# ToniChopp/ECAMP

Hardware: AMD Instinct MI355X
Metric: pretrain image-report pairs/sec (ViT-B/16, 224^2, seq=128) (higher is better)
Workload: dtype bf16

## Files before the change

### ecamp_amd/csrc/gemm.hip

```cpp
#include "common.h"
#include <stdlib.h>
#include <string.h>
#include <stdint.h>
#include <map>
#include <string>
#include <vector>

#include "gemm_args.h"
#include "gemm_q8.h"
#include "gemm_q16.h"

#define BM 128
#define BN 128
#define BK 64

__device__ __forceinline__ int swz(int row) { return (row >> 1) & 7; }

__device__ __forceinline__ void g2r_kc(const bf16_t* P, long ld, int row0, int nrows, int k0, int kend, int tid,
                                       uint4 (&r)[4]) {
#pragma unroll
    for (int i = 0; i < 4; ++i) {
        int c = tid + 256 * i;
        int row = c >> 3, kc = c & 7;
        int gr = row0 + row, gk = k0 + kc * 8;
// ... 856 lines not shown
    if (prof) ecamp_prof_end(stream);
    if (q8_out && !q8) {
        const long n4 = M * N / 4;
        int nb = (int)((n4 + 255) / 256);
        if (nb > 4096) nb = 4096;
        hipLaunchKernelGGL(quant_fp8_delayed_kernel<bf16_t>, dim3(nb), dim3(256), 0, stream, (const bf16_t*)C, q8_scale, (unsigned int*)q8_out, q8_amax_slots, n4);
    }
    ECAMP_LAUNCH_CHECK();
    return 0;
}

struct WgTile { int prob, m0, n0, first, count; };
struct WgRedProb { float* C; long ldc; int M, N; float alpha; int accumulate; const float* alpha_dev; };
struct WgRedArgs { const WgTile* tiles; const float* slabs; int ntiles, pad; WgRedProb p[4]; };
__global__ __launch_bounds__(256) void wgrad_group_reduce_kernel(WgRedArgs a) {
    const int t = blockIdx.x >> 4, chunk = blockIdx.x & 15;
    const WgTile T = a.tiles[t];
    const WgRedProb P = T.prob == 0 ? a.p[0] : T.prob == 1 ? a.p[1] : T.prob == 2 ? a.p[2] : a.p[3];
    const float al = P.alpha_dev ? P.alpha * P.alpha_dev[0] : P.alpha;
#pragma unroll
    for (int j = 0; j < 4; ++j) {
        const int idx = chunk * 1024 + j * 256 + threadIdx.x;
        const int r = idx >> 6, c = (idx & 63) * 4;
        const int gm = T.m0 + r, gn = T.n0 + c;
        if (gm >= P.M || gn >= P.N) continue;
        const float4* src = reinterpret_cast<const float4*>(a.slabs + (long)T.first * 65536) + idx;
        float4 acc = src[0];
        for (int z = 1; z < T.count; ++z) {
            const float4 p = src[(long)z * 16384];
            acc.x += p.x; acc.y += p.y; acc.z += p.z; acc.w += p.w;
        }
        float* c_ = P.C + (long)gm * P.ldc + gn;
        float4 o = P.accumulate ? *reinterpret_cast<float4*>(c_) : make_float4(0.f, 0.f, 0.f, 0.f);
        o.x += al * acc.x; o.y += al * acc.y; o.z += al * acc.z; o.w += al * acc.w;
        *reinterpret_cast<float4*>(c_) = o;
    }
}

struct WgPlan {
    std::vector<Q8ItemRec> items;
    std::vector<int> first;
    std::vector<WgTile> tiles;
    int nitems = 0, nwg = 0, ntiles = 0;
    size_t off_first = 0, off_tiles = 0, bytes = 0;
};
static std::map<std::string, WgPlan> g_wg_plans;

static long wg_tiles(int n, const int64_t* n_out, const int64_t* k_in) {
    long tiles = 0;
    for (int p = 0; p < n; ++p) tiles += (long)ceil_div(n_out[p], 256) * ceil_div(k_in[p], 256);
    return tiles;
}

static const WgPlan* wg_plan(int n, const int64_t* n_out, const int64_t* k_in, const unsigned* has_bias, int64_t rows, int ncu) {
    const int reserve = ecamp_opt(OPT_P8_WGRAD_RESERVE);
    std::string key((const char*)n_out, n * sizeof(int64_t));
    key.append((const char*)k_in, n * sizeof(int64_t)).append((const char*)has_bias, n * sizeof(unsigned)).append((const char*)&rows, 8).append((const char*)&ncu, 4);
    key.append((const char*)&reserve, sizeof(int));
    auto it = g_wg_plans.find(key);
    if (it != g_wg_plans.end()) return &it->second;
    const long KT = (rows + 63) / 64;
    WgPlan pl;
    std::vector<WgTile>& tiles = pl.tiles;
    for (int p = 0; p < n; ++p)
        for (int mb = 0; mb < ceil_div(n_out[p], 256); ++mb)
            for (int nb = 0; nb < ceil_div(k_in[p], 256); ++nb) tiles.push_back({p, mb * 256, nb * 256, 0, 0});
    std::vector<Q8ItemRec>& items = pl.items;
    std::vector<int>& first = pl.first;
    const int plan_mode = ecamp_opt(OPT_WGRAD_PLAN);
    const long T = (long)tiles.size();
    const int cap = p8_bwd_cus();
    long S = (ncu + T / 2) / T;
    while (S > 1 && (T * S > cap || KT / S < 4)) --S;
    if (plan_mode == 1 && S >= 1 && T * S >= ncu / 2 && T * S <= cap) {
        const long P = T * S;
        for (long t = 0; t < T; ++t) { tiles[t].first = (int)(t * S); tiles[t].count = (int)S; }
        std::vector<long> order(P);
        for (long j = 0; j < P; ++j) order[j] = j;
        const long q8 = P / 8, r8 = P % 8;
        for (long w = 0; w < P; ++w) {
            const long xcd = w % 8, slot = w / 8;
            const long j = (xcd < r8 ? xcd * (q8 + 1) : r8 * (q8 + 1) + (xcd - r8) * q8) + slot;
            const long seg = order[j] / T, t = order[j] % T;
            const long k0 = KT * seg / S, k1 = KT * (seg + 1) / S;
            const long kend = k1 * 64 < rows ? k1 * 64 : rows;
            WgTile& Tt = tiles[t];
            first.push_back((int)items.size());
            items.push_back({Tt.prob, Tt.m0, Tt.n0, (int)(k0 * 64), (int)kend, (int)(t * S + seg), (Tt.n0 == 0 && has_bias[Tt.prob]) ? 1 : 0, 0});
        }
    } else {
    const long U = KT / 2;
    const long units = (long)tiles.size() * U;
    long q = (units + ncu - 1) / ncu;
    if (q < 1) q = 1;
    long u = 0;
    while (u < units) {
        first.push_back((int)items.size());
        long take = q < units - u ? q : units - u;
        while (take > 0) {
            const long t = u / U, j0 = u % U, len = take < U - j0 ? take : U - j0;
            WgTile& T = tiles[t];
            if (T.count == 0) T.first = (int)items.size();
            ++T.count;
            const long k0 = 2 * j0, k1 = j0 + len == U ? KT : 2 * (j0 + len);
            const long kend = k1 * 64 < rows ? k1 * 64 : rows;
            items.push_back({T.prob, T.m0, T.n0, (int)(k0 * 64), (int)kend, (int)items.size(), (T.n0 == 0 && has_bias[T.prob]) ? 1 : 0, 0});
            u += len; take -= len;
        }
    }
    }
    first.push_back((int)items.size());
    pl.nitems = (int)items.size(); pl.nwg = (int)first.size() - 1; pl.ntiles = (int)tiles.size();
    pl.off_first = items.size() * sizeof(Q8ItemRec);
    pl.off_tiles = pl.off_first + (first.size() * sizeof(int) + 31) / 32 * 32;
    pl.bytes = pl.off_tiles + tiles.size() * sizeof(WgTile);
    return &(g_wg_plans[key] = std::move(pl));
}
static int wg_ncu() {
    const int env = ecamp_opt(OPT_WGRAD_GROUP_CUS), ncu = p8_num_cu();
    if (env > 0) return env < ncu ? env : ncu;
    const int bwd = p8_bwd_cus(), q = ncu * 3 / 4;
    return bwd < q ? bwd : q;
}
extern "C" int ecamp_wgrad_group_supported(int32_t n, const int64_t* n_out, const int64_t* k_in, int64_t rows) {
    if (n < 1 || n > 4 || !n_out || !k_in || rows < 256) return 0;
    for (int p = 0; p < n; ++p) {
        if (n_out[p] % 8 || k_in[p] % 8 || n_out[p] <= 0 || k_in[p] <= 0) return 0;
        if (rows * n_out[p] * 2 > LIM_2GB || rows * k_in[p] * 2 > LIM_2GB) return 0;
    }
    return wg_tiles(n, n_out, k_in) >= 16 ? 1 : 0;
}
extern "C" int64_t ecamp_wgrad_group_workspace_bytes(int32_t n, const int64_t* n_out, const int64_t* k_in, int64_t rows) {
    if (!ecamp_wgrad_group_supported(n, n_out, k_in, rows)) return 0;
    return (wg_tiles(n, n_out, k_in) + p8_num_cu() + 1) * 262144;
}
extern "C" int ecamp_wgrad_group_workgroups(int32_t workgroups) {
    if (workgroups > 0) return workgroups < p8_num_cu() ? workgroups : p8_num_cu();
    return wg_ncu();
}
extern "C" int64_t ecamp_wgrad_group_table_bytes(int32_t n, const int64_t* n_out, const int64_t* k_in, int64_t rows) {
    if (!ecamp_wgrad_group_supported(n, n_out, k_in, rows)) return 0;
    const long tiles = wg_tiles(n, n_out, k_in), ncu = p8_num_cu();
    return (tiles + ncu + 1) * (long)sizeof(Q8ItemRec) + ((ncu + 2) * 4 + 31) / 32 * 32 + tiles * (long)sizeof(WgTile) + 64;
}
extern "C" int64_t ecamp_wgrad_group_table(int32_t n, const int64_t* n_out, const int64_t* k_in, const int32_t* has_bias, int64_t rows,
                                           int32_t workgroups, void* host_table) {
    if (!n_out || !k_in || !has_bias || !host_table || !ecamp_wgrad_group_supported(n, n_out, k_in, rows))
        return ecamp_set_error(-1, "wgrad_group_table: unsupported group or null pointer");
    unsigned hb[4] = {0, 0, 0, 0};
    for (int p = 0; p < n; ++p) hb[p] = has_bias[p] ? 1u : 0u;
    const WgPlan* pl = wg_plan(n, n_out, k_in, hb, rows, ecamp_wgrad_group_workgroups(workgroups));
    char* out = (char*)host_table;
    memcpy(out, pl->items.data(), pl->items.size() * sizeof(Q8ItemRec));
    memcpy(out + pl->off_first, pl->first.data(), pl->first.size() * sizeof(int));
    memcpy(out + pl->off_tiles, pl->tiles.data(), pl->tiles.size() * sizeof(WgTile));
    return (int64_t)pl->bytes;
}
extern "C" int ecamp_wgrad_group(int32_t n, const void* const* dy, const void* const* x, float* const* gw, float* const* gb, const int64_t* n_out,
                                 const int64_t* k_in, int64_t rows, float alpha, const float* alpha_dev, const int32_t* accumulate, float* ws,
                                 const void* table, int64_t table_bytes, int32_t workgroups, hipStream_t stream) {
    ECAMP_CHECK_ARG(dy && x && gw && gb && n_out && k_in && accumulate && ws && table, "wgrad_group: null pointer");
    ECAMP_CHECK_ARG(((uintptr_t)table & 31) == 0, "wgrad_group: the item table must be 32-byte aligned");
    ECAMP_CHECK_ARG(ecamp_wgrad_group_supported(n, n_out, k_in, rows), "wgrad_group: unsupported group (1-4 layers, rows >= 256, dims %% 8 == 0, < 2 GB operands)");
    unsigned hb[4] = {0, 0, 0, 0};
    bool any_bias = false;
    for (int p = 0; p < n; ++p) {
        ECAMP_CHECK_ARG(dy[p] && x[p] && gw[p], "wgrad_group: null operand");
        ECAMP_CHECK_ARG(((uintptr_t)dy[p] & 15) == 0 && ((uintptr_t)x[p] & 15) == 0 && ((uintptr_t)gw[p] & 15) == 0, "wgrad_group: operands must be 16-byte aligned");
        hb[p] = gb[p] ? 1u : 0u;
        any_bias = any_bias || gb[p];
    }
    const int nwg = ecamp_wgrad_group_workgroups(workgroups);
    const WgPlan* pl = wg_plan(n, n_out, k_in, hb, rows, nwg);
    ECAMP_CHECK_ARG(table_bytes == (int64_t)pl->bytes, "wgrad_group: the item table (%ld bytes) was not built for the current plan (%ld bytes: CU reserve "
                    "or workgroup count changed since ecamp_wgrad_group_table) -- rebuild it", (long)table_bytes, (long)pl->bytes);
    const char* tb = (const char*)table;
    Q8Group G;
    memset(&G, 0, sizeof(G));
    G.items = (const Q8ItemRec*)tb; G.wg_first = (const int*)(tb + pl->off_first); G.slabs = ws; G.nprob = n;
    WgRedArgs R;
    memset(&R, 0, sizeof(R));
    R.tiles = (const WgTile*)(tb + pl->off_tiles); R.slabs = ws; R.ntiles = pl->ntiles;
    for (int p = 0; p < n; ++p) {
        G.p[p].A = dy[p]; G.p[p].B = x[p]; G.p[p].lda = n_out[p]; G.p[p].ldb = k_in[p]; G.p[p].M = (int)n_out[p]; G.p[p].N = (int)k_in[p];
        G.p[p].rowsum = gb[p]; G.p[p].alpha_out = alpha; G.p[p].alpha_dev_out = alpha_dev;
        R.p[p].C = gw[p]; R.p[p].ldc = k_in[p]; R.p[p].M = (int)n_out[p]; R.p[p].N = (int)k_in[p]; R.p[p].alpha = alpha; R.p[p].alpha_dev = alpha_dev;
        R.p[p].accumulate = accumulate[p];
    }
    GemmArgs g = gemm_args(dy[0], x[0], ws, n_out[0], k_in[0], rows, n_out[0], k_in[0], k_in[0]);
    g.out_f32 = 1; g.alpha_out = alpha; g.nbm = 1; g.nbn = 1; g.wide = 1; g.partial = ws;
    typedef void (*q8i_fn)(GemmArgs, Q8Group);
    const bool lean = (ecamp_opt(OPT_Q8_SCH) & 8) != 0;
    const bool four = q16_wgrad_on(Q16W_GROUPED);
    const q8i_fn fn = four ? (any_bias ? (q8i_fn)gemm_bf16_q16_wgrad_items_kernel<true> : (q8i_fn)gemm_bf16_q16_wgrad_items_kernel<false>)
                    : any_bias ? (lean ? (q8i_fn)gemm_bf16_q8_items_kernel<true, 1> : (q8i_fn)gemm_bf16_q8_items_kernel<true, 0>)
                               : (lean ? (q8i_fn)gemm_bf16_q8_items_kernel<false, 1> : (q8i_fn)gemm_bf16_q8_items_kernel<false, 0>);
    double work = 0.0;
    for (int p = 0; p < n; ++p) work += 2.0 * (double)n_out[p] * (double)k_in[p] * (double)rows;
    const bool prof = ecamp_prof_active();
    if (prof) {
        char tag[40];
        snprintf(tag, sizeof tag, "%s:w:n%d:%ld:%ld:%ld:wg%d", four ? "grp16" : "grp", n, (long)rows, (long)n_out[0], (long)k_in[0], pl->nwg);
        ecamp_prof_begin(ECAMP_PROF_GEMM_BF16, work, stream, tag);
    }
    launch_persistent(fn, (long)pl->nwg, (long)pl->nwg, four ? 256 : 512, stream, g, G);
    g_q8_launches += n;
    if (four) ++g_q16_launches;
    ++g_wg_launches;
    hipLaunchKernelGGL(wgrad_group_reduce_kernel, dim3(pl->ntiles * 16), dim3(256), 0, stream, R);
    if (prof) ecamp_prof_end(stream);
    ECAMP_LAUNCH_CHECK();
    return 0;
}
```

### ecamp_amd/functions.py

```python
import math
import os

import torch

from . import hip_ops as ops


def _none(n):
    return (None,) * n


_BLOCK = None


class _wgrad_block:

    def __init__(self, arena):
        self.arena, self.items, self.ready, self.prev = arena, [], [], None

    def __enter__(self):
        global _BLOCK
        self.prev, _BLOCK = _BLOCK, self
        self.outer_ready, self.arena.deferred = self.arena.deferred, self.ready
        return self

    def collect(self, item):
        self.items.append(item)
        if len(self.items) == 4:
            self.issue()

    def issue(self):
        _issue(self.items)
        del self.items[:]

    def __exit__(self, et, ev, tb):
        global _BLOCK
        _BLOCK, self.arena.deferred = self.prev, self.outer_ready
        if et is None:
            self.issue()
            if self.ready:
                self.arena.ready(*self.ready)
        return False


def _issue(items, workgroups=0):
    if len(items) >= 2 and ops.wgrad_group_supported(items):
        ops.wgrad_group_async(items, workgroups=workgroups)
    else:
        for dy, x, gw, gb, acc in items:
            ops.linear_wgrad_async(dy, x, gw, gb=gb, accumulate=acc)


_MLM_CHUNK_ROWS = int(os.environ.get("ECAMP_MLM_CHUNK_ROWS", "0"))


def _wgrad(A, dy, x, w, gb=None, alpha_dev=None, shape=None):
    gw, acc = A.gradw(w, shape)
    if _BLOCK is not None and _BLOCK.arena is A and alpha_dev is None:
        _BLOCK.collect((dy, x, gw, gb, acc))
        return
    ops.linear_wgrad_async(dy, x, gw, alpha_dev=alpha_dev, gb=gb, accumulate=acc)


def _f8_site(m, x, weights):
    if not (m.fp8_forward and x.dtype == torch.bfloat16):
        return None
    _, sc, am, cal = m.arena.f8_site(weights)
    return (sc, am) if cal else None


def _dense(m, x, weights, bias, shape=None, x8=None, next_w=None, **kw):
    A = m.arena
    plist = list(weights) if isinstance(weights, (list, tuple)) else [weights]
    if m.fp8_forward and x.dtype == torch.bfloat16:
        i, sc, am, cal = A.f8_site(plist)
        if x8 is None:
            x8 = ops.quantize_fp8_site(x, sc, am, cal)
            A.f8_cal.add(i)
        w8, ws = A.w8(plist, shape)
        if next_w is not None:
            _, nsc, nam, ncal = A.f8_site(next_w)
            if ncal:
                return ops.gemm_fp8(x8, sc, w8, ws, bias, q8_site=(nsc, nam), **kw)
            return ops.gemm_fp8(x8, sc, w8, ws, bias, **kw) + (None,)
        return ops.gemm_fp8(x8, sc, w8, ws, bias, **kw)
    w = A.fused_w(plist, shape) if len(plist) > 1 else A.w(plist[0])
    r = ops.linear_fwd(x, w, bias, **kw)
    return r + (None,) if next_w is not None else r


def _vit_linear(m, x, lin, x8=None, next_w=None, residual=None, **kw):
    if residual is not None and residual.dtype != x.dtype:
        return ops.linear_fwd_res32(x, m.arena.w(lin.weight), lin.bias.data, residual)
    return _dense(m, x, lin.weight, lin.bias.data, x8=x8, next_w=next_w, residual=residual, **kw)


def f32_carrier(x32, dtype):
    assert x32.dim() == 2 and x32.dtype == torch.float32 and x32.is_contiguous()
    return x32.view(dtype)[:, 0::2]


def f32_stream(x):
    if x.dtype == torch.float32:
        return x
    M, D = x.shape
    assert x.stride() == (2 * D, 2) and x.storage_offset() % 2 == 0, "not an f32 residual-stream carrier"
    return x.new_empty(0, dtype=torch.float32).set_(x.untyped_storage(), x.storage_offset() // 2, (M, D), (D, 1))


def _ln_bwd(dy, z, mean, rstd, gamma, ggamma, gbeta, dres=None):
    if z.dtype != dy.dtype:
# ... 410 lines not shown
    A.ready(ln.weight, ln.bias, out.dense.weight, out.dense.bias, inter.dense.weight, inter.dense.bias)
    return dx


class BertLayerFn(torch.autograd.Function):
    @staticmethod
    def forward(ctx, h, layer, m, B, S, key_mask, pa, ph):
        tape = []
        a, a8 = _self_attn_fwd(m, layer.attention.self, layer.attention.output, h, B, S, key_mask, pa, ph, tape, next_w=layer.intermediate.dense.weight)
        o = _ffn_fwd(m, layer.intermediate, layer.output, a, ph, tape, x8=a8)
        ctx.s = (tape, m, B, S, key_mask, pa, ph)
        return o

    @staticmethod
    def backward(ctx, do):
        tape, m, B, S, key_mask, pa, ph = ctx.s
        with _wgrad_block(m.arena):
            da = _ffn_bwd(m, tape[1], do.contiguous(), ph)
            dh = _self_attn_bwd(m, tape[0], da, B, S, key_mask, pa, ph)
        ctx.s = None
        return (dh,) + _none(7)


class FusionFn(torch.autograd.Function):

    @staticmethod
    def forward(ctx, e, lat, gap, fl, m, B, S, T, key_mask, pa, ph):
        A = m.arena
        H = e.shape[1]
        heads = m.bert_config.num_attention_heads
        hd = H // heads
        tape = []
        a1 = _self_attn_fwd(m, fl.attention.self, fl.attention.output, e, B, S, key_mask, pa, ph, tape)
        ca = fl.cross_self_attention
        q = _dense(m, a1, ca.query.weight, ca.query.bias.data)
        bkv = A.fused_f32([ca.key.bias, ca.value.bias], (2 * H,))
        kv = _dense(m, lat, [ca.key.weight, ca.value.weight], bkv, shape=(2 * H, H))
        f = kv.view(-1)
        qs, ks = (S * H, H, hd), (T * 2 * H, 2 * H, hd)
        s1, o1 = m.next_rng()
        c, lse, cbits = ops.attn_fwd(q, f[2 * H:], f[3 * H:], B, heads, S, T - 1, hd, qs, ks, ks, 1.0 / math.sqrt(hd), None, pa, s1, o1, want_mask=True)
        gp = ops.linear_fwd(gap, A.w(fl.gap_mlp.weight), fl.gap_mlp.bias.data)
        c2 = ops.bcast_add(c, gp).view(B * S, H)
        ol = fl.out_layer
        y = _dense(m, c2, ol.dense.weight, ol.dense.bias.data)
        s2, o2 = m.next_rng()
        a2, z, mean, rstd, a28 = _ln_fwd(m, y, ol.LayerNorm, fl.intermediate.dense.weight, residual=a1, drop_p=ph, seed=s2, offset=o2)
        out = _ffn_fwd(m, fl.intermediate, fl.output, a2, ph, tape, x8=a28)
        ctx.s = (tape, e, lat, gap, fl, m, B, S, T, key_mask, pa, ph, a1, q, kv, c, lse, c2, z, mean, rstd, (s1, o1), (s2, o2), cbits)
        return out

    @staticmethod
    def backward(ctx, dout):
        (tape, e, lat, gap, fl, m, B, S, T, key_mask, pa, ph, a1, q, kv, c, lse, c2, z, mean, rstd, (s1, o1), (s2, o2), cbits) = ctx.s
        A = m.arena
        G = A.grad
        H = e.shape[1]
        heads = m.bert_config.num_attention_heads
        hd = H // heads
        da2 = _ffn_bwd(m, tape[1], dout.contiguous(), ph)
        ol = fl.out_layer
        ln = ol.LayerNorm
        dz, dy = _post_ln_bwd(m, da2, z, mean, rstd, ln, ph, s2, o2)
        _wgrad(A, dy, c2, ol.dense.weight, gb=G(ol.dense.bias))
        dc2 = ops.linear_dgrad(dy, A.w(ol.dense.weight))
        dgp = ops.seq_sum(dc2.view(B, S, H), 0, S, 1.0)
        gm = fl.gap_mlp
        _wgrad(A, dgp, gap, gm.weight, gb=G(gm.bias))
        dgap = ops.linear_dgrad(dgp, A.w(gm.weight))
        ca = fl.cross_self_attention
        dq = torch.empty_like(q)
        dkv = ops.zeros(kv.shape, kv.device, kv.dtype)
        f, df = kv.view(-1), dkv.view(-1)
        qs, ks = (S * H, H, hd), (T * 2 * H, 2 * H, hd)
        ops.attn_bwd(q, f[2 * H:], f[3 * H:], c, dc2.view(B, S, H), lse, dq, df[2 * H:], df[3 * H:], B, heads, S, T - 1, hd, qs, ks, ks,
                     qs, ks, ks, 1.0 / math.sqrt(hd), None, pa, s1, o1, drop_bits=cbits)
        _wgrad(A, dkv, lat, [ca.key.weight, ca.value.weight], shape=(2 * H, H), gb=A.fused_grad([ca.key.bias, ca.value.bias], (2 * H,)))
        dlat = ops.linear_dgrad(dkv, A.fused_w([ca.key.weight, ca.value.weight], (2 * H, H)))
        _wgrad(A, dq, a1, ca.query.weight, gb=G(ca.query.bias))
        da1 = ops.linear_dgrad(dq, A.w(ca.query.weight), residual=dz)
        A.ready(ln.weight, ln.bias, ol.dense.weight, ol.dense.bias, gm.weight, gm.bias, ca.query.weight, ca.query.bias,
                ca.key.weight, ca.key.bias, ca.value.weight, ca.value.bias)
        de = _self_attn_bwd(m, tape[0], da1, B, S, key_mask, pa, ph)
        ctx.s = None
        return (de, dlat, dgap) + _none(8)


def _mlm_transform(m, h, pr):
    fp8 = m.fp8_forward and m.fp8_head
    if fp8:
        t1, pre = _dense(m, h, pr.transform.dense.weight, pr.transform.dense.bias.data, act=1, save_pre=True)
    else:
        t1, pre = ops.linear_fwd(h, m.arena.w(pr.transform.dense.weight), pr.transform.dense.bias.data, act=1, save_pre=True)
    t, _, mean, rstd, t8 = _ln_fwd(m, t1, pr.transform.LayerNorm, pr.decoder.weight if fp8 else None)
    return t1, pre, mean, rstd, t, t8


def _mlm_decoder(m, t, t8, pr):
    if m.fp8_forward and m.fp8_head:
        return _dense(m, t, pr.decoder.weight, pr.bias.data, x8=t8)
    return ops.linear_fwd(t, m.arena.w(pr.decoder.weight), pr.bias.data)


def mlm_head_eval(h, labels, weights, cls, m, ids=None, rows_hint=None, compact=False):
    from .data import MASK
    pr = cls.predictions
    M = h.shape[0]
    labels, weights = labels.view(-1), weights.view(-1)
    ids = ids.view(-1) if ids is not None else None
    m._eval_found = m._aux_mlm_rows = None
    if compact:
        V = pr.decoder.weight.shape[0]
        if rows_hint is None:
            h, labels, weights, rows, found = ops.compact_rows(h, labels, weights, ids, MASK, V, cap=M)
            cap = ops.compact_cap(found.item())
            if cap <= M:
                h, labels, weights, rows = h[:cap], labels[:cap], weights[:cap], rows[:cap]
        else:
            h, labels, weights, rows, found = ops.compact_rows(h, labels, weights, ids, MASK, V, cap=ops.compact_cap(rows_hint))
        m._eval_found = found
        if m.keep_aux:
# ... 131 lines not shown
```

### ecamp_amd/hip_ops.py

```python
import ctypes
import os

import torch

from . import _lib, streams
from ._lib import BF16, F32, call

_I64x3 = ctypes.c_int64 * 3


def code(dtype):
    if dtype == torch.float32:
        return F32
    if dtype == torch.bfloat16 or dtype == torch.float16:
        want = "bf16" if dtype == torch.bfloat16 else "f16"
        if _lib.half() != want:
            raise TypeError("a %s tensor reached the %s build of libecamp_hip -- call ecamp_amd._lib.set_half(%r) first "
                            "(ECAMP(compute_dtype=...) does)" % (dtype, _lib.half(), want))
        return BF16
    raise TypeError("ecamp_amd supports float32, bfloat16 and float16 activations, got %s" % dtype)


def _chk(*ts):
    for t in ts:
# ... 91 lines not shown
        return y, pre, y8
    return (y, pre) if save_pre else y


def linear_fwd_fp8(x, w8, w_scale, bias=None, act=0, residual=None, save_pre=False):
    M, K = x.shape
    N = w8.shape[0]
    assert w8.shape[1] == K and w8.dtype == torch.uint8 and x.dtype == torch.bfloat16 and x.is_contiguous() and w8.is_contiguous()
    x8, xs = quantize_fp8(x)
    y = torch.empty((M, N), device=x.device, dtype=torch.bfloat16)
    pre = torch.empty((M, N), device=x.device, dtype=torch.bfloat16) if save_pre else None
    call("ecamp_gemm_fp8", ptr(x8), ptr(w8), ptr(y), M, N, K, K, K, N, ptr(xs), ptr(w_scale), ptr(bias), ptr(residual),
         residual.stride(0) if residual is not None else 0, ptr(pre), N, int(act), ptr(None), ptr(None), ptr(None), stream())
    return (y, pre) if save_pre else y


def linear_dgrad(dy, w, gmul=None, alpha=1.0, alpha_dev=None, residual=None, gmul_is_grad=False):
    M, N = dy.shape
    K = w.shape[1]
    dx = torch.empty((M, K), device=dy.device, dtype=dy.dtype)
    gemm(dy, w, dx, M, K, N, True, dy.stride(0), False, w.stride(0), K, gmul=gmul, ldg=gmul.stride(0) if gmul is not None else 0,
         residual=residual, ldr=residual.stride(0) if residual is not None else 0, alpha=alpha, alpha_dev=alpha_dev,
         act=2 if (gmul_is_grad and gmul is not None) else 0)
    return dx


_SPLIT_CACHE = {}
_WG_TABLES = {}


def set_option(name, value):
    call("ecamp_set_option", name.encode(), int(value))
    _SPLIT_CACHE.clear()
    _WG_TABLES.clear()


def _split_k(n_out, k_in, m, dtype=torch.bfloat16):
    key = (n_out, k_in, m, dtype)
    s = _SPLIT_CACHE.get(key)
    if s is None:
        s = _SPLIT_CACHE[key] = max(1, int(_lib.load().ecamp_gemm_suggest_split(n_out, k_in, m, 0, 0, code(dtype))))
    return s


def linear_wgrad(dy, x, gw, alpha=1.0, alpha_dev=None, gb=None, accumulate=True):
    M, N = dy.shape
    K = x.shape[1]
    assert gw.dtype == torch.float32 and gw.is_contiguous() and gw.numel() == N * K
    gemm(dy, x, gw, N, K, M, False, dy.stride(0), False, x.stride(0), K, alpha=alpha, alpha_dev=alpha_dev, out_f32=True,
         accumulate=bool(accumulate), split_k=_split_k(N, K, M, dy.dtype), rowsum=gb)


WGRAD_GROUP = os.environ.get("ECAMP_WGRAD_GROUP", "1") != "0"


def wgrad_group_supported(items):
    if not WGRAD_GROUP or not 1 <= len(items) <= 4:
        return False
    rows = items[0][0].shape[0]
    for dy, x, gw, gb, _ in items:
        if dy.dtype not in (torch.bfloat16, torch.float16) or x.dtype != dy.dtype or dy.shape[0] != rows or x.shape[0] != rows:
            return False
        if not (dy.is_contiguous() and x.is_contiguous() and gw.is_contiguous() and gw.dtype == torch.float32):
            return False
    n = len(items)
    no = (ctypes.c_int64 * n)(*[it[0].shape[1] for it in items])
    ki = (ctypes.c_int64 * n)(*[it[1].shape[1] for it in items])
    return bool(_lib.load().ecamp_wgrad_group_supported(n, ctypes.cast(no, ctypes.c_void_p), ctypes.cast(ki, ctypes.c_void_p), rows))


def _wgrad_group_table(dev, n, no, ki, hb, rows, workgroups):
    lib = _lib.load()
    nwg = int(lib.ecamp_wgrad_group_workgroups(int(workgroups)))
    key = (str(dev), tuple(no), tuple(ki), tuple(hb), int(rows), nwg)
    t = _WG_TABLES.get(key)
    if t is None:
        cv = lambda a: ctypes.cast(a, ctypes.c_void_p)
        cap = int(lib.ecamp_wgrad_group_table_bytes(n, cv(no), cv(ki), rows))
        host = torch.empty((cap,), dtype=torch.uint8)
        used = int(lib.ecamp_wgrad_group_table(n, cv(no), cv(ki), cv((ctypes.c_int32 * n)(*hb)), rows, int(workgroups), ctypes.c_void_p(host.data_ptr())))
        if used <= 0:
            raise _lib.EcampHipError("ecamp_wgrad_group_table failed: %s" % lib.ecamp_last_error().decode())
        t = _WG_TABLES[key] = host[:used].to(dev)
    return t


def wgrad_group(items, alpha=1.0, alpha_dev=None, workgroups=0):
    n = len(items)
    rows = items[0][0].shape[0]
    no = (ctypes.c_int64 * n)(*[it[0].shape[1] for it in items])
    ki = (ctypes.c_int64 * n)(*[it[1].shape[1] for it in items])
    vp = lambda ts: (ctypes.c_void_p * n)(*[t.data_ptr() if t is not None else None for t in ts])
    dyp, xp, gwp, gbp = vp([it[0] for it in items]), vp([it[1] for it in items]), vp([it[2] for it in items]), vp([it[3] for it in items])
    acc = (ctypes.c_int32 * n)(*[1 if it[4] else 0 for it in items])
    cv = lambda a: ctypes.cast(a, ctypes.c_void_p)
    dev = items[0][0].device
    table = _wgrad_group_table(dev, n, no, ki, [1 if it[3] is not None else 0 for it in items], rows, workgroups)
    nws = int(_lib.load().ecamp_wgrad_group_workspace_bytes(n, cv(no), cv(ki), rows)) // 4
    ws = torch.empty((nws,), device=dev, dtype=torch.float32)
    call("ecamp_wgrad_group", n, cv(dyp), cv(xp), cv(gwp), cv(gbp), cv(no), cv(ki), rows, float(alpha), ptr(alpha_dev), cv(acc), ptr(ws), ptr(table),
         table.numel(), int(workgroups), stream())


def colsum(x, out, alpha=1.0, period=0, lo=0, hi=0, alpha_dev=None):
    _chk(x, out)
    M, N = x.shape
    call("ecamp_colsum", ptr(x), x.stride(0), M, N, float(alpha), ptr(alpha_dev), period, lo, hi, ptr(out), code(x.dtype), stream())


def layernorm_fwd(x, gamma, beta, eps, residual=None, drop_p=0.0, seed=0, offset=0, q8_site=None):
    _chk(x, gamma, beta)
    rows, cols = x.shape
    assert x.is_contiguous()
    y = torch.empty_like(x)
    mean = torch.empty(rows, device=x.device, dtype=torch.float32)
    rstd = torch.empty(rows, device=x.device, dtype=torch.float32)
    fused = residual is not None or drop_p > 0.0
    z = torch.empty_like(x) if fused else None
    if q8_site is not None:
        y8 = torch.empty((rows, cols), device=x.device, dtype=torch.uint8)
        call("ecamp_layernorm_fwd_q8", ptr(x), ptr(residual), ptr(z), ptr(gamma), ptr(beta), ptr(y), ptr(mean), ptr(rstd), rows, cols,
             float(eps), float(drop_p), seed, offset, ptr(y8), ptr(q8_site[0]), ptr(q8_site[1]), code(x.dtype), stream())
        return y, (z if fused else x), mean, rstd, y8
    call("ecamp_layernorm_fwd", ptr(x), ptr(residual), ptr(z), ptr(gamma), ptr(beta), ptr(y), ptr(mean), ptr(rstd), rows, cols,
         float(eps), float(drop_p), seed, offset, code(x.dtype), stream())
    return y, (z if fused else x), mean, rstd


def layernorm_bwd(dy, z, mean, rstd, gamma, ggamma, gbeta, dres=None, drop_p=0.0, seed=0, offset=0, want_drop=False):
    rows, cols = dy.shape
    assert dy.is_contiguous() and z.is_contiguous()
    dz = torch.empty_like(dy)
    dxd = torch.empty_like(dy) if want_drop else None
    call("ecamp_layernorm_bwd", ptr(dy), ptr(z), ptr(mean), ptr(rstd), ptr(gamma), ptr(dres), ptr(dz), ptr(dxd), ptr(ggamma),
         ptr(gbeta), rows, cols, float(drop_p), seed, offset, code(dy.dtype), stream())
    return (dz, dxd) if want_drop else dz


def layernorm_fwd_x32(x, gamma, beta, eps, dtype):
    _chk(x, gamma, beta)
    rows, cols = x.shape
    assert x.is_contiguous() and x.dtype == torch.float32
    y = torch.empty((rows, cols), device=x.device, dtype=dtype)
    mean = torch.empty(rows, device=x.device, dtype=torch.float32)
    rstd = torch.empty(rows, device=x.device, dtype=torch.float32)
    call("ecamp_layernorm_fwd_x32", ptr(x), ptr(gamma), ptr(beta), ptr(y), ptr(mean), ptr(rstd), rows, cols, float(eps), code(dtype), stream())
    return y, x, mean, rstd


def layernorm_bwd_z32(dy, z, mean, rstd, gamma, ggamma, gbeta, dres=None):
    rows, cols = dy.shape
    assert dy.is_contiguous() and z.is_contiguous() and z.dtype == torch.float32 and (dres is None or dres.dtype == dy.dtype)
    dz = torch.empty_like(dy)
    call("ecamp_layernorm_bwd_z32", ptr(dy), ptr(z), ptr(mean), ptr(rstd), ptr(gamma), ptr(dres), ptr(dz), ptr(ggamma), ptr(gbeta), rows, cols,
# ... 544 lines not shown
```

### include/ecamp_hip.h

```cpp
#ifndef ECAMP_HIP_H
#define ECAMP_HIP_H
#include <stdint.h>
#ifdef __cplusplus
extern "C" {
#endif

typedef struct ihipStream_t* ecampStream_t;

#define ECAMP_F32 0
#define ECAMP_BF16 1

#define ECAMP_ABI_VERSION 5
int ecamp_abi_version(void);
const char* ecamp_last_error(void);
int ecamp_half_format(void);

int ecamp_gemm(const void* A, const void* B, void* C, int64_t M, int64_t N, int64_t K, int a_kc, int64_t lda, int b_kc,
               int64_t ldb, int64_t ldc, const float* bias, const void* residual, int64_t ldr, void* pre_out, int64_t ldp,
               const void* gmul, int64_t ldg, int act, float alpha, const float* alpha_dev, int dtype, int out_f32, int accumulate,
               int split_k, float* splitk_ws, float* rowsum, ecampStream_t stream);
int ecamp_gemm_res32(const void* A, const void* B, float* C, int64_t M, int64_t N, int64_t K, int64_t lda, int64_t ldb, int64_t ldc,
                     const float* bias, const float* residual, int64_t ldr, int dtype, ecampStream_t stream);
int ecamp_gemm_suggest_split(int64_t M, int64_t N, int64_t K, int a_kc, int b_kc, int dtype);
int ecamp_wgrad_group_supported(int32_t n, const int64_t* n_out, const int64_t* k_in, int64_t rows);
int64_t ecamp_wgrad_group_workspace_bytes(int32_t n, const int64_t* n_out, const int64_t* k_in, int64_t rows);
int64_t ecamp_wgrad_group_table_bytes(int32_t n, const int64_t* n_out, const int64_t* k_in, int64_t rows);
int64_t ecamp_wgrad_group_table(int32_t n, const int64_t* n_out, const int64_t* k_in, const int32_t* has_bias, int64_t rows,
                                int32_t workgroups, void* host_table);
int ecamp_wgrad_group_workgroups(int32_t workgroups);
int ecamp_wgrad_group(int32_t n, const void* const* dy, const void* const* x, float* const* gw, float* const* gb, const int64_t* n_out,
                      const int64_t* k_in, int64_t rows, float alpha, const float* alpha_dev, const int32_t* accumulate, float* ws,
                      const void* table, int64_t table_bytes, int32_t workgroups, ecampStream_t stream);
int64_t ecamp_gemm_workspace_bytes(int64_t M, int64_t N, int64_t K, int32_t split_k);
int64_t ecamp_attn_bwd_workspace_bytes(int32_t B, int32_t H, int32_t Tq);
int64_t ecamp_sr_bwd_workspace_bytes(void);
int ecamp_set_option(const char* name, int32_t value);

int ecamp_amax(const void* x, float* out, int64_t n, int32_t dtype, ecampStream_t stream);
int ecamp_quant_fp8_delayed(const void* x, const float* scale, void* q, float* amax_slots, int64_t n, int32_t dtype, ecampStream_t stream);
int ecamp_fp8_roll(float* amax_slots, float* scale, int32_t n, float* hist, int32_t hist_len, int32_t hist_pos, float margin, ecampStream_t stream);
int ecamp_fp8_weights(const void* w_bf16, void* w8, const int32_t* items, int32_t nitems, float* amax_slots, const float* scales,
                      int32_t pass, ecampStream_t stream);
int ecamp_layernorm_fwd_q8(const void* x, const void* residual, void* z_out, const float* gamma, const float* beta, void* y, float* mean,
                           float* rstd, int64_t rows, int32_t cols, float eps, float drop_p, uint64_t seed, uint64_t offset, void* q8,
                           const float* q8_scale, float* q8_amax_slots, int32_t dtype, ecampStream_t stream);
int ecamp_quant_fp8(const void* x, const float* amax, void* q, float* scale_out, int64_t n, int32_t dtype, ecampStream_t stream);
int ecamp_gemm_fp8(const void* A8, const void* B8, void* C, int64_t M, int64_t N, int64_t K, int64_t lda, int64_t ldb, int64_t ldc,
                   const float* scale_a, const float* scale_b, const float* bias, const void* residual, int64_t ldr, void* pre_out,
                   int64_t ldp, int act, void* q8_out, const float* q8_scale, float* q8_amax_slots, ecampStream_t stream);

int ecamp_layernorm_fwd(const void* x, const void* residual, void* z_out, const float* gamma, const float* beta, void* y,
                        float* mean, float* rstd, int64_t rows, int32_t cols, float eps, float drop_p, uint64_t seed,
                        uint64_t offset, int32_t dtype, ecampStream_t stream);
int ecamp_layernorm_bwd(const void* dy, const void* z, const float* mean, const float* rstd, const float* gamma,
                        const void* dres_in, void* dz, void* dx_drop, float* dgamma, float* dbeta, int64_t rows, int32_t cols,
                        float drop_p, uint64_t seed, uint64_t offset, int32_t dtype, ecampStream_t stream);
int ecamp_layernorm_fwd_x32(const float* x, const float* gamma, const float* beta, void* y, float* mean, float* rstd, int64_t rows,
                            int32_t cols, float eps, int32_t dtype, ecampStream_t stream);
int ecamp_layernorm_bwd_z32(const void* dy, const float* z, const float* mean, const float* rstd, const float* gamma, const void* dres_in,
                            void* dz, float* dgamma, float* dbeta, int64_t rows, int32_t cols, int32_t dtype, ecampStream_t stream);
int ecamp_layernorm_layout(int32_t backward, int32_t rows16, int32_t cols, int32_t al16, int32_t opt_bwd, int32_t* out);

int64_t ecamp_attn_mask_bytes(int32_t B, int32_t H, int32_t Tq, int32_t Tk, int32_t hd, int32_t dtype);
int ecamp_attn_fwd(const void* q, const void* k, const void* v, void* o, float* lse, const int32_t* key_mask, int32_t B,
                   int32_t H, int32_t Tq, int32_t Tk, int32_t hd, const int64_t* q_strides, const int64_t* k_strides,
                   const int64_t* v_strides, const int64_t* o_strides, float scale, float drop_p, uint64_t seed, uint64_t offset,
                   int32_t dtype, void* drop_mask, ecampStream_t stream);
int ecamp_attn_bwd(const void* q, const void* k, const void* v, const void* o, const void* dout, const float* lse,
                   float* delta_ws, void* dq, void* dk, void* dv, const int32_t* key_mask, int32_t B, int32_t H, int32_t Tq,
                   int32_t Tk, int32_t hd, const int64_t* q_strides, const int64_t* k_strides, const int64_t* v_strides,
                   const int64_t* o_strides, const int64_t* do_strides, const int64_t* dq_strides, const int64_t* dk_strides,
                   const int64_t* dv_strides, float scale, float drop_p, uint64_t seed, uint64_t offset, int32_t dtype,
                   const void* drop_mask, ecampStream_t stream);
int ecamp_attn_probs(const void* q, const void* k, const int32_t* key_mask, float* probs, int32_t B, int32_t H, int32_t Tq, int32_t Tk,
                     int32_t hd, const int64_t* q_strides, const int64_t* k_strides, float scale, int32_t dtype, ecampStream_t stream);

int ecamp_add(const void* a, const void* b, void* y, int64_t n, int32_t dtype, ecampStream_t stream);
int ecamp_gelu_bwd(const void* dy, const void* pre, void* dx, int64_t n, int32_t dtype, ecampStream_t stream);
int ecamp_cast(const void* src, void* dst, int64_t n, int32_t src_dtype, int32_t dst_dtype, ecampStream_t stream);
int ecamp_scale(const void* x, void* y, int64_t n, float alpha, const float* alpha_dev, int32_t dtype, ecampStream_t stream);
int ecamp_zero(void* p, int64_t bytes, ecampStream_t stream);
int ecamp_colsum(const void* X, int64_t ld, int64_t M, int64_t N, float alpha, const float* alpha_dev, int32_t period, int32_t lo, int32_t hi,
                 float* out, int32_t dtype, ecampStream_t stream);
int ecamp_bcast_add(const void* x, const void* g, void* y, int64_t B, int32_t S, int32_t H, int32_t dtype,
                    ecampStream_t stream);
// ... 131 lines not shown
```

Baseline: 7391.

## Allow grouped weight-gradient GEMMs with different row counts per layer

Extends the grouped wgrad planner and API so each problem in a group can have its own row count. K-splitting becomes per-problem and is balanced by k-tile work, with a loop that adds splits to the longest piece while within the CU cap. The Python side now permits mixed-row groups and adds an optional fusion-block grouping for the fusion backward, which is off by default via ECAMP_WGRAD_FUSION_GROUP=0. The per-problem split heuristic also changes the plan for equal-row groups, which can shift load balance in the default path.

```diff
diff --git a/ecamp_amd/csrc/gemm.hip b/ecamp_amd/csrc/gemm.hip
--- a/ecamp_amd/csrc/gemm.hip
+++ b/ecamp_amd/csrc/gemm.hip
@@ -932,14 +932,18 @@
     return tiles;
 }
 
-static const WgPlan* wg_plan(int n, const int64_t* n_out, const int64_t* k_in, const unsigned* has_bias, int64_t rows, int ncu) {
+static const WgPlan* wg_plan(int n, const int64_t* n_out, const int64_t* k_in, const unsigned* has_bias, const int64_t* rows, int ncu) {
     const int reserve = ecamp_opt(OPT_P8_WGRAD_RESERVE);
     std::string key((const char*)n_out, n * sizeof(int64_t));
-    key.append((const char*)k_in, n * sizeof(int64_t)).append((const char*)has_bias, n * sizeof(unsigned)).append((const char*)&rows, 8).append((const char*)&ncu, 4);
-    key.append((const char*)&reserve, sizeof(int));
+    key.append((const char*)k_in, n * sizeof(int64_t)).append((const char*)has_bias, n * sizeof(unsigned)).append((const char*)rows, n * sizeof(int64_t));
+    key.append((const char*)&ncu, 4).append((const char*)&reserve, sizeof(int));
     auto it = g_wg_plans.find(key);
     if (it != g_wg_plans.end()) return &it->second;
-    const long KT = (rows + 63) / 64;
+    long KT[4] = {0, 0, 0, 0}, Tp[4] = {0, 0, 0, 0};
+    for (int p = 0; p < n; ++p) {
+        KT[p] = (rows[p] + 63) / 64;
+        Tp[p] = (long)ceil_div(n_out[p], 256) * ceil_div(k_in[p], 256);
+    }
     WgPlan pl;
     std::vector<WgTile>& tiles = pl.tiles;
     for (int p = 0; p < n; ++p)
@@ -950,42 +954,74 @@
     const int plan_mode = ecamp_opt(OPT_WGRAD_PLAN);
     const long T = (long)tiles.size();
     const int cap = p8_bwd_cus();
-    long S = (ncu + T / 2) / T;
-    while (S > 1 && (T * S > cap || KT / S < 4)) --S;
-    if (plan_mode == 1 && S >= 1 && T * S >= ncu / 2 && T * S <= cap) {
-        const long P = T * S;
-        for (long t = 0; t < T; ++t) { tiles[t].first = (int)(t * S); tiles[t].count = (int)S; }
-        std::vector<long> order(P);
-        for (long j = 0; j < P; ++j) order[j] = j;
+    long ktiles = 0, S[4] = {0, 0, 0, 0};
+    for (int p = 0; p < n; ++p) ktiles += Tp[p] * KT[p];
+    for (int p = 0; p < n; ++p) {
+        S[p] = (2 * KT[p] * ncu + ktiles) / (2 * ktiles);
+        if (S[p] > KT[p] / 4) S[p] = KT[p] / 4;
+        if (S[p] < 1) S[p] = 1;
+    }
+    auto pieces = [&]() { long c = 0; for (int p = 0; p < n; ++p) c += Tp[p] * S[p]; return c; };
+    for (bool any = true; any && pieces() > cap;) {
+        any = false;
+        for (int p = 0; p < n; ++p)
+            if (S[p] > 1) { --S[p]; any = true; }
+    }
+    for (;;) {
+        int own = 0;
+        long longest = 0;
+        for (int p = 0; p < n; ++p) {
+            const long len = (KT[p] + S[p] - 1) / S[p];
+            if (len > longest) { longest = len; own = p; }
+        }
+        const long P = pieces();
+        if (4 * longest * P <= 5 * ktiles || S[own] + 1 > KT[own] / 4 || P + Tp[own] > cap) break;
+        ++S[own];
+    }
+    const long P = pieces();
+    if (plan_mode == 1 && T <= 2L * ncu && P >= ncu / 2 && P <= cap) {
+        long slab = 0, smax = 0;
+        for (long t = 0; t < T; ++t) {
+            tiles[t].first = (int)slab; tiles[t].count = (int)S[tiles[t].prob];
+            slab += S[tiles[t].prob];
+        }
+        for (int p = 0; p < n; ++p) smax = S[p] > smax ? S[p] : smax;
+        std::vector<long> order;
+        order.reserve(P);
+        for (long seg = 0; seg < smax; ++seg)
+            for (long t = 0; t < T; ++t)
+                if (seg < S[tiles[t].prob]) order.push_back(seg * T + t);
         const long q8 = P / 8, r8 = P % 8;
         for (long w = 0; w < P; ++w) {
             const long xcd = w % 8, slot = w / 8;
             const long j = (xcd < r8 ? xcd * (q8 + 1) : r8 * (q8 + 1) + (xcd - r8) * q8) + slot;
             const long seg = order[j] / T, t = order[j] % T;
-            const long k0 = KT * seg / S, k1 = KT * (seg + 1) / S;
-            const long kend = k1 * 64 < rows ? k1 * 64 : rows;
             WgTile& Tt = tiles[t];
+            const long kt = KT[Tt.prob], s = S[Tt.prob];
+            const long k0 = kt * seg / s, k1 = kt * (seg + 1) / s;
+            const long kend = k1 * 64 < rows[Tt.prob] ? k1 * 64 : rows[Tt.prob];
             first.push_back((int)items.size());
-            items.push_back({Tt.prob, Tt.m0, Tt.n0, (int)(k0 * 64), (int)kend, (int)(t * S + seg), (Tt.n0 == 0 && has_bias[Tt.prob]) ? 1 : 0, 0});
+            items.push_back({Tt.prob, Tt.m0, Tt.n0, (int)(k0 * 64), (int)kend, Tt.first + (int)seg, (Tt.n0 == 0 && has_bias[Tt.prob]) ? 1 : 0, 0});
         }
     } else {
-    const long U = KT / 2;
-    const long units = (long)tiles.size() * U;
+    long units = 0;
+    for (int p = 0; p < n; ++p) units += Tp[p] * (KT[p] / 2);
     long q = (units + ncu - 1) / ncu;
     if (q < 1) q = 1;
-    long u = 0;
+    long u = 0, t = 0, j0 = 0;
     while (u < units) {
         first.push_back((int)items.size());
         long take = q < units - u ? q : units - u;
         while (take > 0) {
-            const long t = u / U, j0 = u % U, len = take < U - j0 ? take : U - j0;
             WgTile& T = tiles[t];
+            const long U = KT[T.prob] / 2, len = take < U - j0 ? take : U - j0;
             if (T.count == 0) T.first = (int)items.size();
             ++T.count;
-            const long k0 = 2 * j0, k1 = j0 + len == U ? KT : 2 * (j0 + len);
-            const long kend = k1 * 64 < rows ? k1 * 64 : rows;
+            const long k0 = 2 * j0, k1 = j0 + len == U ? KT[T.prob] : 2 * (j0 + len);
+            const long kend = k1 * 64 < rows[T.prob] ? k1 * 64 : rows[T.prob];
             items.push_back({T.prob, T.m0, T.n0, (int)(k0 * 64), (int)kend, (int)items.size(), (T.n0 == 0 && has_bias[T.prob]) ? 1 : 0, 0});
-            u += len; take -= len;
+            u += len; take -= len; j0 += len;
+            if (j0 == U) { ++t; j0 = 0; }
         }
     }
     }
@@ -1002,30 +1038,31 @@
     const int bwd = p8_bwd_cus(), q = ncu * 3 / 4;
     return bwd < q ? bwd : q;
 }
-extern "C" int ecamp_wgrad_group_supported(int32_t n, const int64_t* n_out, const int64_t* k_in, int64_t rows) {
-    if (n < 1 || n > 4 || !n_out || !k_in || rows < 256) return 0;
+extern "C" int ecamp_wgrad_group_rows_supported(int32_t n, const int64_t* n_out, const int64_t* k_in, const int64_t* rows) {
+    if (n < 1 || n > 4 || !n_out || !k_in || !rows) return 0;
     for (int p = 0; p < n; ++p) {
+        if (rows[p] < 256) return 0;
         if (n_out[p] % 8 || k_in[p] % 8 || n_out[p] <= 0 || k_in[p] <= 0) return 0;
-        if (rows * n_out[p] * 2 > LIM_2GB || rows * k_in[p] * 2 > LIM_2GB) return 0;
+        if (rows[p] * n_out[p] * 2 > LIM_2GB || rows[p] * k_in[p] * 2 > LIM_2GB) return 0;
     }
     return wg_tiles(n, n_out, k_in) >= 16 ? 1 : 0;
 }
-extern "C" int64_t ecamp_wgrad_group_workspace_bytes(int32_t n, const int64_t* n_out, const int64_t* k_in, int64_t rows) {
-    if (!ecamp_wgrad_group_supported(n, n_out, k_in, rows)) return 0;
+extern "C" int64_t ecamp_wgrad_group_rows_workspace_bytes(int32_t n, const int64_t* n_out, const int64_t* k_in, const int64_t* rows) {
+    if (!ecamp_wgrad_group_rows_supported(n, n_out, k_in, rows)) return 0;
     return (wg_tiles(n, n_out, k_in) + p8_num_cu() + 1) * 262144;
 }
 extern "C" int ecamp_wgrad_group_workgroups(int32_t workgroups) {
     if (workgroups > 0) return workgroups < p8_num_cu() ? workgroups : p8_num_cu();
     return wg_ncu();
 }
-extern "C" int64_t ecamp_wgrad_group_table_bytes(int32_t n, const int64_t* n_out, const int64_t* k_in, int64_t rows) {
-    if (!ecamp_wgrad_group_supported(n, n_out, k_in, rows)) return 0;
+extern "C" int64_t ecamp_wgrad_group_rows_table_bytes(int32_t n, const int64_t* n_out, const int64_t* k_in, const int64_t* rows) {
+    if (!ecamp_wgrad_group_rows_supported(n, n_out, k_in, rows)) return 0;
     const long tiles = wg_tiles(n, n_out, k_in), ncu = p8_num_cu();
     return (tiles + ncu + 1) * (long)sizeof(Q8ItemRec) + ((ncu + 2) * 4 + 31) / 32 * 32 + tiles * (long)sizeof(WgTile) + 64;
 }
-extern "C" int64_t ecamp_wgrad_group_table(int32_t n, const int64_t* n_out, const int64_t* k_in, const int32_t* has_bias, int64_t rows,
-                                           int32_t workgroups, void* host_table) {
-    if (!n_out || !k_in || !has_bias || !host_table || !ecamp_wgrad_group_supported(n, n_out, k_in, rows))
+extern "C" int64_t ecamp_wgrad_group_rows_table(int32_t n, const int64_t* n_out, const int64_t* k_in, const int32_t* has_bias, const int64_t* rows,
+                                                int32_t workgroups, void* host_table) {
+    if (!n_out || !k_in || !has_bias || !host_table || !ecamp_wgrad_group_rows_supported(n, n_out, k_in, rows))
         return ecamp_set_error(-1, "wgrad_group_table: unsupported group or null pointer");
     unsigned hb[4] = {0, 0, 0, 0};
     for (int p = 0; p < n; ++p) hb[p] = has_bias[p] ? 1u : 0u;
@@ -1036,12 +1073,29 @@
     memcpy(out + pl->off_tiles, pl->tiles.data(), pl->tiles.size() * sizeof(WgTile));
     return (int64_t)pl->bytes;
 }
-extern "C" int ecamp_wgrad_group(int32_t n, const void* const* dy, const void* const* x, float* const* gw, float* const* gb, const int64_t* n_out,
-                                 const int64_t* k_in, int64_t rows, float alpha, const float* alpha_dev, const int32_t* accumulate, float* ws,
-                                 const void* table, int64_t table_bytes, int32_t workgroups, hipStream_t stream) {
-    ECAMP_CHECK_ARG(dy && x && gw && gb && n_out && k_in && accumulate && ws && table, "wgrad_group: null pointer");
+struct WgRows {
+    int64_t r[4];
+    WgRows(int32_t n, int64_t rows) { for (int p = 0; p < 4; ++p) r[p] = p < n ? rows : 0; }
+};
+extern "C" int ecamp_wgrad_group_supported(int32_t n, const int64_t* n_out, const int64_t* k_in, int64_t rows) {
+    return ecamp_wgrad_group_rows_supported(n, n_out, k_in, WgRows(n, rows).r);
+}
+extern "C" int64_t ecamp_wgrad_group_workspace_bytes(int32_t n, const int64_t* n_out, const int64_t* k_in, int64_t rows) {
+    return ecamp_wgrad_group_rows_workspace_bytes(n, n_out, k_in, WgRows(n, rows).r);
+}
+extern "C" int64_t ecamp_wgrad_group_table_bytes(int32_t n, const int64_t* n_out, const int64_t* k_in, int64_t rows) {
+    return ecamp_wgrad_group_rows_table_bytes(n, n_out, k_in, WgRows(n, rows).r);
+}
+extern "C" int64_t ecamp_wgrad_group_table(int32_t n, const int64_t* n_out, const int64_t* k_in, const int32_t* has_bias, int64_t rows,
+                                           int32_t workgroups, void* host_table) {
+    return ecamp_wgrad_group_rows_table(n, n_out, k_in, has_bias, WgRows(n, rows).r, workgroups, host_table);
+}
+extern "C" int ecamp_wgrad_group_rows(int32_t n, const void* const* dy, const void* const* x, float* const* gw, float* const* gb, const int64_t* n_out,
+                                      const int64_t* k_in, const int64_t* rows, float alpha, const float* alpha_dev, const int32_t* accumulate, float* ws,
+                                      const void* table, int64_t table_bytes, int32_t workgroups, hipStream_t stream) {
+    ECAMP_CHECK_ARG(dy && x && gw && gb && n_out && k_in && rows && accumulate && ws && table, "wgrad_group: null pointer");
     ECAMP_CHECK_ARG(((uintptr_t)table & 31) == 0, "wgrad_group: the item table must be 32-byte aligned");
-    ECAMP_CHECK_ARG(ecamp_wgrad_group_supported(n, n_out, k_in, rows), "wgrad_group: unsupported group (1-4 layers, rows >= 256, dims %% 8 == 0, < 2 GB operands)");
+    ECAMP_CHECK_ARG(ecamp_wgrad_group_rows_supported(n, n_out, k_in, rows), "wgrad_group: unsupported group (1-4 layers, rows >= 256 each, dims %% 8 == 0, < 2 GB operands)");
     unsigned hb[4] = {0, 0, 0, 0};
     bool any_bias = false;
     for (int p = 0; p < n; ++p) {
@@ -1052,8 +1106,8 @@
     }
     const int nwg = ecamp_wgrad_group_workgroups(workgroups);
     const WgPlan* pl = wg_plan(n, n_out, k_in, hb, rows, nwg);
-    ECAMP_CHECK_ARG(table_bytes == (int64_t)pl->bytes, "wgrad_group: the item table (%ld bytes) was not built for the current plan (%ld bytes: CU reserve "
-                    "or workgroup count changed since ecamp_wgrad_group_table) -- rebuild it", (long)table_bytes, (long)pl->bytes);
+    ECAMP_CHECK_ARG(table_bytes == (int64_t)pl->bytes, "wgrad_group: the item table (%ld bytes) was not built for the current plan (%ld bytes: CU reserve, "
+                    "workgroup count or row counts changed since ecamp_wgrad_group_table) -- rebuild it", (long)table_bytes, (long)pl->bytes);
     const char* tb = (const char*)table;
     Q8Group G;
     memset(&G, 0, sizeof(G));
@@ -1067,7 +1121,7 @@
         R.p[p].C = gw[p]; R.p[p].ldc = k_in[p]; R.p[p].M = (int)n_out[p]; R.p[p].N = (int)k_in[p]; R.p[p].alpha = alpha; R.p[p].alpha_dev = alpha_dev;
         R.p[p].accumulate = accumulate[p];
     }
-    GemmArgs g = gemm_args(dy[0], x[0], ws, n_out[0], k_in[0], rows, n_out[0], k_in[0], k_in[0]);
+    GemmArgs g = gemm_args(dy[0], x[0], ws, n_out[0], k_in[0], rows[0], n_out[0], k_in[0], k_in[0]);
     g.out_f32 = 1; g.alpha_out = alpha; g.nbm = 1; g.nbn = 1; g.wide = 1; g.partial = ws;
     typedef void (*q8i_fn)(GemmArgs, Q8Group);
     const bool lean = (ecamp_opt(OPT_Q8_SCH) & 8) != 0;
@@ -1076,11 +1130,11 @@
                     : any_bias ? (lean ? (q8i_fn)gemm_bf16_q8_items_kernel<true, 1> : (q8i_fn)gemm_bf16_q8_items_kernel<true, 0>)
                                : (lean ? (q8i_fn)gemm_bf16_q8_items_kernel<false, 1> : (q8i_fn)gemm_bf16_q8_items_kernel<false, 0>);
     double work = 0.0;
-    for (int p = 0; p < n; ++p) work += 2.0 * (double)n_out[p] * (double)k_in[p] * (double)rows;
+    for (int p = 0; p < n; ++p) work += 2.0 * (double)n_out[p] * (double)k_in[p] * (double)rows[p];
     const bool prof = ecamp_prof_active();
     if (prof) {
         char tag[40];
-        snprintf(tag, sizeof tag, "%s:w:n%d:%ld:%ld:%ld:wg%d", four ? "grp16" : "grp", n, (long)rows, (long)n_out[0], (long)k_in[0], pl->nwg);
+        snprintf(tag, sizeof tag, "%s:w:n%d:%ld:%ld:%ld:wg%d", four ? "grp16" : "grp", n, (long)rows[0], (long)n_out[0], (long)k_in[0], pl->nwg);
         ecamp_prof_begin(ECAMP_PROF_GEMM_BF16, work, stream, tag);
     }
     launch_persistent(fn, (long)pl->nwg, (long)pl->nwg, four ? 256 : 512, stream, g, G);
@@ -1092,3 +1146,8 @@
     ECAMP_LAUNCH_CHECK();
     return 0;
 }
+extern "C" int ecamp_wgrad_group(int32_t n, const void* const* dy, const void* const* x, float* const* gw, float* const* gb, const int64_t* n_out,
+                                 const int64_t* k_in, int64_t rows, float alpha, const float* alpha_dev, const int32_t* accumulate, float* ws,
+                                 const void* table, int64_t table_bytes, int32_t workgroups, hipStream_t stream) {
+    return ecamp_wgrad_group_rows(n, dy, x, gw, gb, n_out, k_in, WgRows(n, rows).r, alpha, alpha_dev, accumulate, ws, table, table_bytes, workgroups, stream);
+}
diff --git a/ecamp_amd/functions.py b/ecamp_amd/functions.py
--- a/ecamp_amd/functions.py
+++ b/ecamp_amd/functions.py
@@ -54,9 +54,9 @@
 _MLM_CHUNK_ROWS = int(os.environ.get("ECAMP_MLM_CHUNK_ROWS", "0"))
 
 
-def _wgrad(A, dy, x, w, gb=None, alpha_dev=None, shape=None):
+def _wgrad(A, dy, x, w, gb=None, alpha_dev=None, shape=None, alone=False):
     gw, acc = A.gradw(w, shape)
-    if _BLOCK is not None and _BLOCK.arena is A and alpha_dev is None:
+    if _BLOCK is not None and _BLOCK.arena is A and alpha_dev is None and not alone:
         _BLOCK.collect((dy, x, gw, gb, acc))
         return
     ops.linear_wgrad_async(dy, x, gw, alpha_dev=alpha_dev, gb=gb, accumulate=acc)
@@ -573,6 +573,13 @@
 
     @staticmethod
     def backward(ctx, dout):
+        if not ops.WGRAD_FUSION_GROUP:
+            return FusionFn._backward(ctx, dout)
+        with _wgrad_block(ctx.s[5].arena):
+            return FusionFn._backward(ctx, dout)
+
+    @staticmethod
+    def _backward(ctx, dout):
         (tape, e, lat, gap, fl, m, B, S, T, key_mask, pa, ph, a1, q, kv, c, lse, c2, z, mean, rstd, (s1, o1), (s2, o2), cbits) = ctx.s
         A = m.arena
         G = A.grad
@@ -587,7 +594,7 @@
         dc2 = ops.linear_dgrad(dy, A.w(ol.dense.weight))
         dgp = ops.seq_sum(dc2.view(B, S, H), 0, S, 1.0)
         gm = fl.gap_mlp
-        _wgrad(A, dgp, gap, gm.weight, gb=G(gm.bias))
+        _wgrad(A, dgp, gap, gm.weight, gb=G(gm.bias), alone=True)
         dgap = ops.linear_dgrad(dgp, A.w(gm.weight))
         ca = fl.cross_self_attention
         dq = torch.empty_like(q)
diff --git a/ecamp_amd/hip_ops.py b/ecamp_amd/hip_ops.py
--- a/ecamp_amd/hip_ops.py
+++ b/ecamp_amd/hip_ops.py
@@ -167,54 +167,57 @@
 
 
 WGRAD_GROUP = os.environ.get("ECAMP_WGRAD_GROUP", "1") != "0"
+WGRAD_FUSION_GROUP = os.environ.get("ECAMP_WGRAD_FUSION_GROUP", "0") == "1"
+
+
+def _wgrad_group_dims(items):
+    n = len(items)
+    return (n, (ctypes.c_int64 * n)(*[it[0].shape[1] for it in items]), (ctypes.c_int64 * n)(*[it[1].shape[1] for it in items]),
+            (ctypes.c_int64 * n)(*[it[0].shape[0] for it in items]))
 
 
 def wgrad_group_supported(items):
     if not WGRAD_GROUP or not 1 <= len(items) <= 4:
         return False
-    rows = items[0][0].shape[0]
     for dy, x, gw, gb, _ in items:
-        if dy.dtype not in (torch.bfloat16, torch.float16) or x.dtype != dy.dtype or dy.shape[0] != rows or x.shape[0] != rows:
+        if dy.dtype not in (torch.bfloat16, torch.float16) or x.dtype != dy.dtype or x.shape[0] != dy.shape[0]:
             return False
         if not (dy.is_contiguous() and x.is_contiguous() and gw.is_contiguous() and gw.dtype == torch.float32):
             return False
-    n = len(items)
-    no = (ctypes.c_int64 * n)(*[it[0].shape[1] for it in items])
-    ki = (ctypes.c_int64 * n)(*[it[1].shape[1] for it in items])
-    return bool(_lib.load().ecamp_wgrad_group_supported(n, ctypes.cast(no, ctypes.c_void_p), ctypes.cast(ki, ctypes.c_void_p), rows))
+    n, no, ki, rows = _wgrad_group_dims(items)
+    cv = lambda a: ctypes.cast(a, ctypes.c_void_p)
+    return bool(_lib.load().ecamp_wgrad_group_rows_supported(n, cv(no), cv(ki), cv(rows)))
 
 
 def _wgrad_group_table(dev, n, no, ki, hb, rows, workgroups):
     lib = _lib.load()
     nwg = int(lib.ecamp_wgrad_group_workgroups(int(workgroups)))
-    key = (str(dev), tuple(no), tuple(ki), tuple(hb), int(rows), nwg)
+    key = (str(dev), tuple(no), tuple(ki), tuple(hb), tuple(rows), nwg)
     t = _WG_TABLES.get(key)
     if t is None:
         cv = lambda a: ctypes.cast(a, ctypes.c_void_p)
-        cap = int(lib.ecamp_wgrad_group_table_bytes(n, cv(no), cv(ki), rows))
+        cap = int(lib.ecamp_wgrad_group_rows_table_bytes(n, cv(no), cv(ki), cv(rows)))
         host = torch.empty((cap,), dtype=torch.uint8)
-        used = int(lib.ecamp_wgrad_group_table(n, cv(no), cv(ki), cv((ctypes.c_int32 * n)(*hb)), rows, int(workgroups), ctypes.c_void_p(host.data_ptr())))
+        used = int(lib.ecamp_wgrad_group_rows_table(n, cv(no), cv(ki), cv((ctypes.c_int32 * n)(*hb)), cv(rows), int(workgroups),
+                                                    ctypes.c_void_p(host.data_ptr())))
         if used <= 0:
-            raise _lib.EcampHipError("ecamp_wgrad_group_table failed: %s" % lib.ecamp_last_error().decode())
+            raise _lib.EcampHipError("ecamp_wgrad_group_rows_table failed: %s" % lib.ecamp_last_error().decode())
         t = _WG_TABLES[key] = host[:used].to(dev)
     return t
 
 
 def wgrad_group(items, alpha=1.0, alpha_dev=None, workgroups=0):
-    n = len(items)
-    rows = items[0][0].shape[0]
-    no = (ctypes.c_int64 * n)(*[it[0].shape[1] for it in items])
-    ki = (ctypes.c_int64 * n)(*[it[1].shape[1] for it in items])
+    n, no, ki, rows = _wgrad_group_dims(items)
     vp = lambda ts: (ctypes.c_void_p * n)(*[t.data_ptr() if t is not None else None for t in ts])
     dyp, xp, gwp, gbp = vp([it[0] for it in items]), vp([it[1] for it in items]), vp([it[2] for it in items]), vp([it[3] for it in items])
     acc = (ctypes.c_int32 * n)(*[1 if it[4] else 0 for it in items])
     cv = lambda a: ctypes.cast(a, ctypes.c_void_p)
     dev = items[0][0].device
     table = _wgrad_group_table(dev, n, no, ki, [1 if it[3] is not None else 0 for it in items], rows, workgroups)
-    nws = int(_lib.load().ecamp_wgrad_group_workspace_bytes(n, cv(no), cv(ki), rows)) // 4
+    nws = int(_lib.load().ecamp_wgrad_group_rows_workspace_bytes(n, cv(no), cv(ki), cv(rows))) // 4
     ws = torch.empty((nws,), device=dev, dtype=torch.float32)
-    call("ecamp_wgrad_group", n, cv(dyp), cv(xp), cv(gwp), cv(gbp), cv(no), cv(ki), rows, float(alpha), ptr(alpha_dev), cv(acc), ptr(ws), ptr(table),
-         table.numel(), int(workgroups), stream())
+    call("ecamp_wgrad_group_rows", n, cv(dyp), cv(xp), cv(gwp), cv(gbp), cv(no), cv(ki), cv(rows), float(alpha), ptr(alpha_dev), cv(acc), ptr(ws),
+         ptr(table), table.numel(), int(workgroups), stream())
 
 
 def colsum(x, out, alpha=1.0, period=0, lo=0, hi=0, alpha_dev=None):
diff --git a/include/ecamp_hip.h b/include/ecamp_hip.h
--- a/include/ecamp_hip.h
+++ b/include/ecamp_hip.h
@@ -31,6 +31,14 @@
 int ecamp_wgrad_group(int32_t n, const void* const* dy, const void* const* x, float* const* gw, float* const* gb, const int64_t* n_out,
                       const int64_t* k_in, int64_t rows, float alpha, const float* alpha_dev, const int32_t* accumulate, float* ws,
                       const void* table, int64_t table_bytes, int32_t workgroups, ecampStream_t stream);
+int ecamp_wgrad_group_rows_supported(int32_t n, const int64_t* n_out, const int64_t* k_in, const int64_t* rows);
+int64_t ecamp_wgrad_group_rows_workspace_bytes(int32_t n, const int64_t* n_out, const int64_t* k_in, const int64_t* rows);
+int64_t ecamp_wgrad_group_rows_table_bytes(int32_t n, const int64_t* n_out, const int64_t* k_in, const int64_t* rows);
+int64_t ecamp_wgrad_group_rows_table(int32_t n, const int64_t* n_out, const int64_t* k_in, const int32_t* has_bias, const int64_t* rows,
+                                     int32_t workgroups, void* host_table);
+int ecamp_wgrad_group_rows(int32_t n, const void* const* dy, const void* const* x, float* const* gw, float* const* gb, const int64_t* n_out,
+                           const int64_t* k_in, const int64_t* rows, float alpha, const float* alpha_dev, const int32_t* accumulate, float* ws,
+                           const void* table, int64_t table_bytes, int32_t workgroups, ecampStream_t stream);
 int64_t ecamp_gemm_workspace_bytes(int64_t M, int64_t N, int64_t K, int32_t split_k);
 int64_t ecamp_attn_bwd_workspace_bytes(int32_t B, int32_t H, int32_t Tq);
 int64_t ecamp_sr_bwd_workspace_bytes(void);
```

After: 7391. Within noise of the previous version (-0.0%).
